# YuliangXiu/ICON

Measured on NVIDIA H100. Metric: M query-points/sec at 256^3 grid, higher is better.
Workload: dtype f32

## Files before the change

### icon_b200/_C.py

```python
import ctypes
import os

_HERE = os.path.dirname(os.path.abspath(__file__))
LIB_PATH = os.environ.get("ICON_B200_LIB") or os.path.join(_HERE, "libicon_b200.so")

if not os.path.exists(LIB_PATH):
    raise ImportError(
        f"{LIB_PATH} is missing: the CUDA extension must be built (python -m icon_b200.build); "
        "icon_b200 has no CPU or PyTorch fallback.")

lib = ctypes.CDLL(LIB_PATH)

_vp, _i, _i64, _f, _sz = ctypes.c_void_p, ctypes.c_int, ctypes.c_int64, ctypes.c_float, ctypes.c_size_t

_SIGS = {
    "icon_version": (_i, []),
    "icon_last_error": (ctypes.c_char_p, []),
    "icon_launch_count": (_i64, []),
    "icon_profile_enable": (_i, [_i]),
    "icon_profile_last_query": (_i, [_vp]),
    "icon_smpl_workspace_bytes": (_sz, [_i, _i]),
    "icon_smpl_prepare": (_i, [_vp, _vp, _vp, _vp, _i, _i, _vp, _sz, _vp]),
    "icon_query_workspace_bytes": (_sz, [_i64, _i, _i]),
    "icon_set_mlp_impl": (_i, [_i]),
    "icon_get_mlp_impl": (_i, []),
    "icon_query": (_i, [_i, _vp, _i64, _i64, _i64, _vp, _vp, _i, _i, _i, _vp, _i, _vp, _i, _i, _vp, _vp, _i, _f,
                        _vp, _vp, _sz, _vp]),
    "icon_query_feats": (_i, [_i, _vp, _i64, _i64, _i64, _vp, _vp, _i, _i, _i, _vp, _i, _vp, _i, _i, _vp, _vp, _i, _f,
                              _i, _vp, _vp, _sz, _vp]),
    "icon_set_sdf_policy": (_i, [_i, _i64, _i64]),
    "icon_set_sdf_bricks": (_i, [_i, _i64]),
    "icon_sdf_brick_info": (_i, [_vp, _i, _i, _vp]),
    "icon_sdf_brick_lists": (_i, [_vp, _i, _i, _vp, _vp, _vp, _vp, _vp, _vp, _vp]),
    "icon_sdf_only": (_i, [_vp, _i64, _i64, _i64, _vp, _vp, _i, _i, _vp, _vp, _vp, _sz, _vp]),
    "icon_sdf_bruteforce": (_i, [_vp, _i64, _i64, _i64, _vp, _vp, _i, _i, _vp, _vp, _vp]),
    "icon_mesh_workspace_bytes": (_sz, [_i, _i]),
    "icon_mesh_prepare": (_i, [_vp, _vp, _i, _i, _vp, _sz, _vp]),
    "icon_mesh_distance": (_i, [_vp, _i64, _vp, _i, _i, _vp, _vp, _vp]),
    "icon_mesh_sample_workspace_bytes": (_sz, [_i]),
    "icon_mesh_sample": (_i, [_vp, _vp, _i, _i, _vp, _i, ctypes.c_uint64, _vp, _vp, _vp, _vp, _sz, _vp]),
    "icon_prt_workspace_bytes": (_sz, [_i, _i, _i]),
    "icon_prt": (_i, [_vp, _i, _i, _vp, _vp, _i, ctypes.c_double, _vp, _vp, _i, _i, ctypes.c_double, _vp, _vp, _vp, _sz,
                      _vp]),
    "icon_mlp_only": (_i, [_vp, _i, _i64, _vp, _vp, _vp, _vp]),
# ... 135 lines not shown
```

### icon_b200/csrc/common.cu

```cuda
#include <stdarg.h>
#include <atomic>

#include <stdlib.h>

#include "common.cuh"

namespace icon {

static thread_local char g_err[512] = "";
static std::atomic<int64_t> g_launches{0};

void set_error(const char *fmt, ...) {
    va_list ap;
    va_start(ap, fmt);
    vsnprintf(g_err, sizeof(g_err), fmt, ap);
    va_end(ap);
}
void count_launch(int n) { g_launches += n; }

constexpr int SCAN_T = 1024, SCAN_I = 4, SCAN_B = SCAN_T * SCAN_I;

__global__ void __launch_bounds__(SCAN_T) k_scan_block(const int32_t *__restrict__ in,
                                                       int32_t *__restrict__ out, int64_t n,
                                                       int32_t *__restrict__ block_sums,
// ... 64 lines not shown
        return ICON_OK;
    }
    int64_t nb = (n + SCAN_B - 1) / SCAN_B;
    if (nb == 1) {
        k_scan_block<<<1, SCAN_T, 0, stream>>>(in, out, n, nullptr, d_total);
        ICON_LAUNCHED();
        return ICON_OK;
    }
    int32_t *sums = (int32_t *)ws;
    void *next_ws = (char *)ws + align_up((size_t)nb * sizeof(int32_t), 256);
    k_scan_block<<<(unsigned)nb, SCAN_T, 0, stream>>>(in, out, n, sums, nullptr);
    ICON_LAUNCHED();
    int rc = scan_exclusive_i32(sums, sums, nb, d_total, next_ws, stream);
    if (rc) return rc;
    k_scan_add<<<(unsigned)nb, SCAN_T, 0, stream>>>(out, n, sums);
    ICON_LAUNCHED();
    return ICON_OK;
}


__global__ void k_csr_count(const int32_t *__restrict__ own, int64_t n, int32_t *__restrict__ cnt) {
    const int64_t i = (int64_t)blockIdx.x * blockDim.x + threadIdx.x;
    if (i < n && own[i] >= 0) atomicAdd(&cnt[own[i]], 1);
}

__global__ void k_csr_fill(const int32_t *__restrict__ own, const int32_t *__restrict__ key, int64_t n,
                           const int32_t *__restrict__ off, int32_t *__restrict__ cursor, int32_t *__restrict__ list) {
    const int64_t i = (int64_t)blockIdx.x * blockDim.x + threadIdx.x;
    if (i < n && own[i] >= 0) list[off[own[i]] + atomicAdd(&cursor[own[i]], 1)] = key[i];
}
// ... 135 lines not shown
```

### icon_b200/csrc/common.cuh

```cuda
#pragma once
#include <cuda_runtime.h>
#include <stdint.h>
#include <stdio.h>

#include "../../include/icon_b200.h"

namespace icon {

void set_error(const char *fmt, ...);
void count_launch(int n = 1);

#define ICON_CHECK_ARG(cond, ...)                 \
    do {                                          \
        if (!(cond)) {                            \
            icon::set_error(__VA_ARGS__);         \
            return ICON_EINVAL;                   \
        }                                         \
    } while (0)

#define ICON_CUDA(expr)                                                              \
    do {                                                                             \
        cudaError_t _e = (expr);                                                     \
        if (_e != cudaSuccess) {                                                     \
            icon::set_error("%s:%d %s -> %s", __FILE__, __LINE__, #expr,             \
// ... 148 lines not shown
    unsigned short *flist;
    float *fkey;
    int64_t face_cap;
    int V;
};
size_t mesh_ws_bytes(int V, int F);
MeshView mesh_view(const void *ws, int V, int F);
void bricks_forget(const MeshView &m);

void profile_mark(int i, cudaStream_t stream);

size_t scan_ws_bytes(int64_t n);
int scan_exclusive_i32(const int32_t *in, int32_t *out, int64_t n, int64_t *d_total ,
                       void *ws, cudaStream_t stream);

struct CsrWs {
    int32_t *cnt, *cursor;
    void *scan_ws;
};
CsrWs csr_take(Carver &c, int64_t rows);
int csr_build(const int32_t *own, const int32_t *key, int64_t n, int R, int32_t *off, int32_t *list, int32_t *ucnt,
              const CsrWs &w, cudaStream_t stream);

size_t vertex_corners_ws_bytes(int V, int F);
int vertex_corners(const int64_t *faces, int F, int V, int32_t *off, int32_t *list, void *ws, cudaStream_t stream);

template <class Fn>
__device__ __forceinline__ void for_each_pass_corner(const int32_t *corners, int n, Fn &&fn) {
    for (int pass = 0; pass < 3; ++pass) {
        const int c = (pass + 1) % 3;
// ... 11 lines not shown
```

### icon_b200/csrc/mlp.cu

```cuda
#include "common.cuh"
#include "query_common.cuh"

namespace icon {

constexpr int MP = 64;
constexpr int MT = 256;
constexpr int KC = 16;

constexpr int OFF_W0 = 0;
constexpr int OFF_B0 = OFF_W0 + 16 * 512;
constexpr int OFF_W1 = OFF_B0 + 512;
constexpr int OFF_B1 = OFF_W1 + 512 * 256;
constexpr int OFF_W2 = OFF_B1 + 256;
constexpr int OFF_B2 = OFF_W2 + 272 * 128;
constexpr int OFF_W3 = OFF_B2 + 128;
constexpr int OFF_B3 = OFF_W3 + 144;
static_assert(OFF_B3 + 1 == ICON_MLP_PACKED_FLOATS, "packed layout");

template <int MODE>
__global__ void __launch_bounds__(MT, 2) k_query_mlp(QueryParams q) {
    extern __shared__ __align__(16) float sm[];
    float *x0s = sm;
    float *stage = sm + 16 * MP;
    float *h1s = stage + 10240;
// ... 213 lines not shown
    __syncthreads();
    if (tid < MP) {
        const int64_t pi = p0 + tid;
        if (pi < q.N) {
            float s = 0.f;
#pragma unroll
            for (int w = 0; w < 8; ++w) s += red[w * MP + tid];
            for (int j = 0; j < 16; ++j) s = fmaf(__ldg(W + OFF_W3 + 128 + j), x0s[j * MP + tid], s);
            s += __ldg(W + OFF_B3);
            float in_cube = (MODE == 3) ? 1.f : q.xyz4[pi].w;
            q.out[pi] = in_cube * s;
        }
    }
}

__global__ void k_outlier_flag(const float *__restrict__ rec, int64_t N, float clip, int32_t *__restrict__ flag) {
    int64_t i = (int64_t)blockIdx.x * blockDim.x + threadIdx.x;
    if (i < N) flag[i] = fabsf(rec[8 * i]) >= clip ? 1 : 0;
}
__global__ void k_outlier_signs(const float *__restrict__ rec, int64_t N, float clip,
                                const int32_t *__restrict__ krank, int8_t *__restrict__ signs) {
    int64_t i = (int64_t)blockIdx.x * blockDim.x + threadIdx.x;
    if (i < N) {
        float s = rec[8 * i];
        if (fabsf(s) >= clip) signs[krank[i]] = s > 0.f ? 1 : -1;
    }
}

constexpr size_t MLP_SMEM = (16 * MP + 10240 + 256 * MP) * sizeof(float);

template <int MODE>
static int launch_mlp(const QueryParams &q, cudaStream_t stream) {
    static bool attr_set[ICON_MAX_DEVICES] = {};
    if (device_needs_setup(attr_set))
        ICON_CUDA(cudaFuncSetAttribute(k_query_mlp<MODE>, cudaFuncAttributeMaxDynamicSharedMemorySize, (int)MLP_SMEM));
    unsigned nblk = (unsigned)((q.N + MP - 1) / MP);
    k_query_mlp<MODE><<<nblk, MT, MLP_SMEM, stream>>>(q);
    ICON_LAUNCHED();
    return ICON_OK;
}

int launch_mlp_tc(int mode, const QueryParams &q, const void *blob, cudaStream_t stream);
static int g_mlp_impl = 1;
// ... 5 lines not shown
            set_error("icon_query / icon_mlp_only: the tensor-core MLP needs the packed tensor-core weight blob (mlp_tc == NULL); "
                      "pass it or select the FP32 kernel with icon_set_mlp_impl(0)");
            return ICON_EINVAL;
        }
        if (q.c0 > 15) {
            set_error("icon_query / icon_mlp_only: the tensor-core MLP takes c0 <= 15 input channels (got %d)", q.c0);
            return ICON_EINVAL;
        }
        return launch_mlp_tc(MODE, q, tc, stream);
    }
    return launch_mlp<MODE>(q, stream);
}

size_t sdf_ws_bytes(int64_t N);
int run_sdf(const float *points, int64_t sc, int64_t sn, int64_t N, const float *h_calib, const MeshView &m,
            float *rec, int32_t *face, void *ws, float4 **xyz4_out, cudaStream_t stream);
int run_points_only(const float *points, int64_t sc, int64_t sn, int64_t N, const float *h_calib,
                    float4 *xyz4, cudaStream_t stream);

struct QueryWs {
    void *sdf_ws;
    float *rec;
    int32_t *krank;
    int8_t *signs;
    int64_t *d_K;
    void *scan_ws;
    float4 *xyz4;
};

static QueryWs carve_query(Carver &c, int64_t N, int prior) {
    QueryWs w{};
    if (prior == ICON_PRIOR_ICON) {
        w.sdf_ws = c.take<char>(sdf_ws_bytes(N));
        w.rec = c.take<float>((size_t)N * 8);
        w.krank = c.take<int32_t>((size_t)N);
        w.signs = c.take<int8_t>((size_t)N);
        w.d_K = c.take<int64_t>(1);
        w.scan_ws = c.take<char>(scan_ws_bytes(N));
    } else {
        w.xyz4 = c.take<float4>((size_t)N);
    }
    return w;
}

}

using namespace icon;

extern "C" size_t icon_query_workspace_bytes(int64_t N, int F, int prior) {
    (void)F;
    Carver c(nullptr);
    carve_query(c, N, prior);
    return c.total();
// ... 34 lines not shown
    q.feat = feat; q.C = C; q.H = H; q.W = W; q.vol = vol_feat; q.VD = VD;
    q.mlp = mlp_packed; q.c0 = c0; q.clip = sdf_clip; q.out = out; q.N = N;
    if (prior == ICON_PRIOR_ICON) {
        ICON_CHECK_ARG(mesh_ws && V > 0 && F > 0, "icon_query: icon prior needs a prepared body mesh");
        ICON_CHECK_ARG((smpl_feats & ~ICON_FEAT_ALL) == 0, "icon_query: smpl_feats mask %d has bits outside ICON_FEAT_ALL",
                       smpl_feats);
        const int cm = smpl_feats & ICON_FEAT_CMAP ? 1 : 0, nm = smpl_feats & ICON_FEAT_NORM ? 1 : 0;
        const bool vs = smpl_feats & ICON_FEAT_VIS;
        const int tail = 1 + 3 * cm + 3 * nm;
        ICON_CHECK_ARG((!vs || C % 2 == 0) && c0 == (vs ? C / 2 : C) + tail,
                       "icon_query: icon prior with smpl_feats mask %d expects c0 = %s + %d (C=%d c0=%d)", smpl_feats,
                       vs ? "C/2" : "C", tail, C, c0);
        q.feats = smpl_feats;
        MeshView m = mesh_view(mesh_ws, V, F);
        float4 *xyz4 = nullptr;
        int rc = run_sdf(points, stride_c, stride_n, N, h_calib, m, w.rec, nullptr, w.sdf_ws, &xyz4, stream);
        if (rc) return rc;
        if (cm) {
            unsigned nb = (unsigned)((N + 255) / 256);
            k_outlier_flag<<<nb, 256, 0, stream>>>(w.rec, N, sdf_clip, w.krank);
            ICON_LAUNCHED();
            rc = scan_exclusive_i32(w.krank, w.krank, N, w.d_K, w.scan_ws, stream);
            if (rc) return rc;
            k_outlier_signs<<<nb, 256, 0, stream>>>(w.rec, N, sdf_clip, w.krank, w.signs);
            ICON_LAUNCHED();
            q.krank = w.krank; q.signs = w.signs; q.d_K = w.d_K;
        }
        q.xyz4 = xyz4; q.rec = w.rec;
        profile_mark(3, stream);
        rc = launch_any<0>(q, mlp_tc, stream);
        profile_mark(4, stream);
        return rc;
    }
    profile_mark(0, stream);
    int rc = run_points_only(points, stride_c, stride_n, N, h_calib, w.xyz4, stream);
    if (rc) return rc;
    profile_mark(1, stream); profile_mark(2, stream); profile_mark(3, stream);
    q.xyz4 = w.xyz4;
    if (prior == ICON_PRIOR_PIFU) {
        ICON_CHECK_ARG(C + 1 == c0, "icon_query: pifu prior expects c0 = C + 1 (C=%d c0=%d)", C, c0);
        rc = launch_any<1>(q, mlp_tc, stream);
        profile_mark(4, stream);
        return rc;
    }
    if (prior == ICON_PRIOR_PAMIR) {
        ICON_CHECK_ARG(vol_feat && VD >= 2 && C + 7 == c0, "icon_query: pamir prior expects vol_feat and c0 = C + 7");
        rc = launch_any<2>(q, mlp_tc, stream);
        profile_mark(4, stream);
        return rc;
    }
    set_error("icon_query: unknown prior %d", prior);
    return ICON_EINVAL;
}

extern "C" int icon_set_mlp_impl(int impl) {
    ICON_CHECK_ARG(impl == 0 || impl == 1, "icon_set_mlp_impl: 0 (fp32) or 1 (tensor cores)");
    g_mlp_impl = impl;
    return ICON_OK;
}
extern "C" int icon_get_mlp_impl(void) { return g_mlp_impl; }

extern "C" int icon_mlp_only(const float *feature, int c0, int64_t N, const float *mlp_packed, const void *mlp_tc,
                             float *out, icon_stream_t stream_) {
    cudaStream_t stream = (cudaStream_t)stream_;
    if (N == 0) return ICON_OK;
    ICON_CHECK_ARG(feature && mlp_packed && out && c0 >= 1 && c0 <= 16, "icon_mlp_only: bad argument");
    QueryParams q{};
    q.raw = feature; q.mlp = mlp_packed; q.c0 = c0; q.out = out; q.N = N;
    return launch_any<3>(q, mlp_tc, stream);
// ... 2 lines not shown
```

### icon_b200/csrc/sdf.cu

```cuda
#include <float.h>

#include <algorithm>
#include <mutex>
#include <type_traits>
#include <unordered_set>
#include <vector>

#include "common.cuh"
#include "face_tree.cuh"
#include "geom.cuh"

namespace icon {

struct Calib {
    float r[9];
    float t[3];
};

__device__ __forceinline__ V3 load_point(const float *__restrict__ pts, int64_t sc, int64_t sn,
                                         int64_t i, const Calib &cb) {
    float px = pts[i * sn], py = pts[sc + i * sn], pz = pts[2 * sc + i * sn];
    V3 o;
    o.x = fmaf(cb.r[2], pz, fmaf(cb.r[1], py, cb.r[0] * px)) + cb.t[0];
    o.y = fmaf(cb.r[5], pz, fmaf(cb.r[4], py, cb.r[3] * px)) + cb.t[1];
    o.z = fmaf(cb.r[8], pz, fmaf(cb.r[7], py, cb.r[6] * px)) + cb.t[2];
    return o;
}

__device__ __forceinline__ void emit_record(V3 p, int bi, float best, int hits, const MeshView &m,
                                            float *__restrict__ rec, int32_t *__restrict__ face,
                                            int64_t idx) {
    Tri t = load_tri(m.tri + 3 * (size_t)bi);
    V3 n = cross3(t.ab, t.ac);
    float s = n.x * n.x + n.y * n.y + n.z * n.z;
    if (s == 0.f) s = 1e-6f;
    float inv = 1.0f / s;
    V3 w = sub3(p, t.a);
    V3 uw = cross3(t.ab, w), wv = cross3(w, t.ac);
    float b2 = (uw.x * n.x + uw.y * n.y + uw.z * n.z) * inv;
    float b1 = (wv.x * n.x + wv.y * n.y + wv.z * n.z) * inv;
    float b0 = 1.0f - b1 - b2;
    const float4 *at = m.attr + 6 * (size_t)bi;
    float4 a0 = __ldg(at), a1 = __ldg(at + 1), a2 = __ldg(at + 2), a3 = __ldg(at + 3),
           a4 = __ldg(at + 4), a5 = __ldg(at + 5);
    float nx = (a0.x * b0 + a0.w * b1 + a1.z * b2) * -1.f;
    float ny = (a0.y * b0 + a1.x * b1 + a1.w * b2) * 1.f;
    float nz = (a0.z * b0 + a1.y * b1 + a2.x * b2) * -1.f;
    float cx = a2.y * b0 + a3.x * b1 + a3.w * b2;
    float cy = a2.z * b0 + a3.y * b1 + a4.x * b2;
    float cz = a2.w * b0 + a3.z * b1 + a4.y * b2;
    float vv = a4.z * b0 + a4.w * b1 + a5.x * b2;
    float vis = vv >= 0.1f ? 1.f : 0.f;
    float dist = sqrtf(best) / sqrtf(3.0f);
    float sign = 2.0f * ((float)(hits & 1) - 0.5f);
    float sdf = dist * sign;
    float4 *r = (float4 *)(rec + 8 * idx);
    r[0] = make_float4(sdf, cx, cy, cz);
    r[1] = make_float4(nx, ny, nz, vis);
    if (face) face[idx] = bi;
}

constexpr int SW_T = 128;
constexpr int NBIN_AX = 128;
constexpr int NBIN = NBIN_AX * NBIN_AX * NBIN_AX;
__host__ __device__ constexpr int fr_cap(int ppw) { return ppw >= 16 ? 1024 : (ppw >= 4 ? 768 : 384); }

__device__ __forceinline__ unsigned spread7(unsigned v) {
    v = (v | (v << 16)) & 0x030000FFu;
    v = (v | (v << 8)) & 0x0300F00Fu;
    v = (v | (v << 4)) & 0x030C30C3u;
    v = (v | (v << 2)) & 0x09249249u;
    return v;
}

// ... 13 lines not shown
    int b = -1;
    if (live) {
        const V3 p = load_point(pts, sc, sn, i, cb);
        const float in_cube = (p.x > -1.f && p.x < 1.f && p.y > -1.f && p.y < 1.f && p.z > -1.f && p.z < 1.f) ? 1.f : 0.f;
        xyz4[i] = make_float4(p.x, p.y, p.z, in_cube);
        b = bin_of(p);
        bid[i] = b;
    }
    const unsigned act = __ballot_sync(0xffffffffu, live);
    if (live) {
        const unsigned peers = __match_any_sync(act, b);
        if ((int)(threadIdx.x & 31) == __ffs(peers) - 1) atomicAdd(&count[b], __popc(peers));
    }
}

__global__ void k_points_scatter(const int32_t *__restrict__ bid, int64_t N, const int32_t *__restrict__ offset,
                                 int32_t *__restrict__ cursor, int32_t *__restrict__ perm) {
    const int64_t i = (int64_t)blockIdx.x * blockDim.x + threadIdx.x;
    const bool live = i < N;
    const int b = live ? bid[i] : -1;
    const unsigned act = __ballot_sync(0xffffffffu, live);
    if (live) {
        const unsigned peers = __match_any_sync(act, b);
        const int lane = threadIdx.x & 31, leader = __ffs(peers) - 1;
        int base = 0;
        if (lane == leader) base = atomicAdd(&cursor[b], __popc(peers));
        base = __shfl_sync(peers, base, leader);
        perm[offset[b] + base + __popc(peers & ((1u << lane) - 1u))] = (int32_t)i;
    }
}

#ifdef ICON_SDF_STATS
__device__ unsigned long long g_stats[8];
__device__ unsigned *g_wstat;
enum { WS_DEFER, WS_ENTRIES, WS_STEPS, WS_STAGED, WS_SPH, WS_EXACT, WS_WIN, WS_RAY, WS_CYC_START, WS_CYC_C,
       WS_CYC_RAY, WS_CYC_EMIT, WS_UB0, WS_UBEND, WS_LIST, WS_IDEAL_ENTRIES, WS_IDEAL_FACES, WS_DEAD, WS_N = 20 };
#define STAT(i, v) do { if (lane == 0) atomicAdd(&g_stats[i], (unsigned long long)(v)); } while (0)
#define WSTAT(i, v) do { if (lane == 0 && g_wstat) g_wstat[(size_t)wid * WS_N + (i)] = (unsigned)(v); } while (0)
#define WCLK(t) __syncwarp(); const long long t = clock64()
#else
#define STAT(i, v) do { } while (0)
#define WSTAT(i, v) do { } while (0)
#endif
// ... 12 lines not shown
    hi = make_float4(-1.f + (bx + 1) * BRICK_W, -1.f + (by + 1) * BRICK_W, -1.f + (bz + 1) * BRICK_W, 0.f);
}

__device__ __forceinline__ float leaf_key(const MeshView &m, int l, float4 lo, float4 hi) {
    const float4 a = __ldg(m.nodes + 2 * (size_t)l), z = __ldg(m.nodes + 2 * (size_t)l + 1);
    const float gx = fmaxf(fmaxf(a.x - hi.x, lo.x - z.x), 0.f);
    const float gy = fmaxf(fmaxf(a.y - hi.y, lo.y - z.y), 0.f);
    const float gz = fmaxf(fmaxf(a.z - hi.z, lo.z - z.z), 0.f);
    return fmaf(gz, gz, fmaf(gy, gy, gx * gx));
}

template <int PPW, bool BRICK>
__device__ __forceinline__ void sdf_warp(int64_t wid, SdfSmem<PPW, BRICK> &S, const float4 *__restrict__ xyz4,
                                         const int32_t *__restrict__ perm, int64_t N, const MeshView &m,
                                         float *__restrict__ rec, int32_t *__restrict__ face,
                                         int32_t *__restrict__ defer, int32_t *__restrict__ ndefer) {
    constexpr int REP = 32 / PPW;
    const int lane = threadIdx.x & 31;
    const int sub = lane % PPW, rep_id = lane / PPW;
    const int64_t pos0 = wid * PPW;
    const int64_t pos = pos0 + sub;
    if (pos0 >= N) return;
    const bool live = pos < N;
    const int64_t idx = perm[live ? pos : pos0];
    const float4 q = xyz4[idx];
    const V3 p = mk3(q.x, q.y, q.z);
    const V3 c = mk3(0.5f * (warp_min(p.x) + warp_max(p.x)), 0.5f * (warp_min(p.y) + warp_max(p.y)),
                     0.5f * (warp_min(p.z) + warp_max(p.z)));
    const float rw = warp_max(sqrtf(dot3(sub3(p, c), sub3(p, c)))) * 1.00001f + 1e-6f;
    const float4 wlo = make_float4(warp_min(p.x) - 1e-6f, warp_min(p.y) - 1e-6f, warp_min(p.z) - 1e-6f, 0.f);
// ... 77 lines not shown
        }
    } else {
        for (int f = rep_id; f < m.F; f += REP) {
            const Tri tr = load_tri(m.tri + 3 * (size_t)f);
            hits += ray_hit_px(p, tr.a, tr.ab, tr.ac);
        }
    }
    if (REP > 1) {
#pragma unroll
        for (int o = PPW; o < 32; o <<= 1) hits += __shfl_xor_sync(0xffffffffu, hits, o);
    }
#ifdef ICON_SDF_STATS
    WCLK(t_ray0);
    t_ray = t_ray0;
#endif
    if (live && rep_id == 0) emit_record(p, nf.bi, nf.best, hits, m, rec, face, idx);
#ifdef ICON_SDF_STATS
    WCLK(t_end);
    if (BRICK && st_brick >= 0) {
        const float ube = nf.ub;
        int il = 0, ifc = 0;
        const int o0 = __ldg(m.foff + st_brick), o1 = __ldg(m.foff + st_brick + 1);
        for (int s = o0 + lane; s < o1; s += 32) {
            il += __ldg(m.fkey + s) <= ube * ube;
            const float4 s4 = __ldg(m.sph_s + __ldg(m.flist + s));
            const float l2 = ube + s4.w;
            ifc += box_dist2(mk3(s4.x, s4.y, s4.z), wlo, whi) <= l2 * l2;
        }
        const int s_sph = __reduce_add_sync(0xffffffffu, nf.n_sph), s_exact = __reduce_add_sync(0xffffffffu, nf.n_exact);
        const int s_win = __reduce_add_sync(0xffffffffu, nf.n_win), s_ray = __reduce_add_sync(0xffffffffu, st_ray);
        const int s_il = __reduce_add_sync(0xffffffffu, il), s_if = __reduce_add_sync(0xffffffffu, ifc);
// ... 10 lines not shown
        WSTAT(WS_CYC_EMIT, t_end - t_ray);
        WSTAT(WS_UB0, __float_as_uint(st_ub0));
        WSTAT(WS_UBEND, __float_as_uint(ube));
        WSTAT(WS_LIST, o1 - o0);
        WSTAT(WS_IDEAL_ENTRIES, s_il);
        WSTAT(WS_IDEAL_FACES, s_if);
        WSTAT(WS_DEAD, nf.n_dead);
    }
    if (!BRICK && defer != nullptr) { STAT(4, 1); STAT(5, t_end - t_start); }
#endif
}

template <int PPW, bool BRICK>
__global__ void __launch_bounds__(SW_T, PPW == 32 ? 8 : 0) k_sdf_warp(const float4 *__restrict__ xyz4, const int32_t *__restrict__ perm,
                                                   int64_t N, MeshView m, float *__restrict__ rec,
                                                   int32_t *__restrict__ face, int32_t *__restrict__ defer,
                                                   int32_t *__restrict__ ndefer) {
    static_assert(!BRICK || PPW == 32, "brick lists serve dense lattices: 32 points per warp");
    extern __shared__ __align__(16) unsigned char smem_raw[];
    SdfSmem<PPW, BRICK> &S = reinterpret_cast<SdfSmem<PPW, BRICK> *>(smem_raw)[threadIdx.x >> 5];
    const bool listed = !BRICK && defer != nullptr;
    const int64_t nw = listed ? (int64_t)*ndefer : (N + PPW - 1) / PPW;
    for (int64_t i = (int64_t)blockIdx.x * (SW_T / 32) + (threadIdx.x >> 5); i < nw; i += (int64_t)gridDim.x * (SW_T / 32))
        sdf_warp<PPW, BRICK>(listed ? (int64_t)defer[i] : i, S, xyz4, perm, N, m, rec, face, defer, ndefer);
}

__global__ void k_brick_centres(MeshView m) {
    const int b = blockIdx.x * blockDim.x + threadIdx.x;
    if (b >= NBRICK) return;
    float4 lo, hi;
    brick_box(b, lo, hi);
    m.bxyz[b] = make_float4(0.5f * (lo.x + hi.x), 0.5f * (lo.y + hi.y), 0.5f * (lo.z + hi.z), 0.f);
    m.bperm[b] = b;
}

template <class Take, class Put>
__device__ __forceinline__ int block_gather(int n, int *s_n, Take &&take, Put &&put) {
    __syncthreads();
    for (int i = threadIdx.x; i < n; i += blockDim.x) {
// ... 133 lines not shown
    for (int f0 = 0; f0 < m.F; f0 += 256) {
        int nf = min(256, m.F - f0);
        __syncthreads();
        for (int k = threadIdx.x; k < 3 * nf; k += 256) tile[k] = m.tri[3 * (size_t)f0 + k];
        __syncthreads();
        if (live) {
            for (int k = 0; k < nf; ++k) {
                float4 r0 = tile[3 * k], r1 = tile[3 * k + 1], r2 = tile[3 * k + 2];
                V3 a = mk3(r0.x, r0.y, r0.z), ab = mk3(r0.w, r1.x, r1.y), ac = mk3(r1.z, r1.w, r2.x);
                float d = tri_sqdist(p, a, ab, ac);
                if (d < best) { best = d; bi = f0 + k; }
                hits += ray_hit_px(p, a, ab, ac);
            }
        }
    }
    if (live) emit_record(p, bi, best, hits, m, rec, face, i);
}

static int64_t g_sdf_ppw32_from = 6000000, g_sdf_ppw8_from = 300000;
static int g_sdf_ppw_force = 0;
static int g_sdf_bricks = 1;
static int64_t g_brick_max_entries = 0;

static std::mutex g_brick_mu;
static std::unordered_set<const void *> g_brick_ready;
static int64_t g_brick_builds = 0;

void bricks_forget(const MeshView &m) {
    std::lock_guard<std::mutex> lk(g_brick_mu);
    g_brick_ready.erase(m.hdr);
}
// ... 10 lines not shown
    w.bid = c.take<int32_t>((size_t)N);
    w.perm = c.take<int32_t>((size_t)N);
    w.count = c.take<int32_t>(NBIN + 1);
    w.offset = c.take<int32_t>(NBIN + 1);
    w.defer = c.take<int32_t>((size_t)(N + 31) / 32);
    w.ndefer = c.take<int32_t>(1);
    w.scan_ws = c.take<char>(scan_ws_bytes(NBIN + 1));
    return w;
}

static int build_bricks(const MeshView &m, cudaStream_t stream) {
    const int64_t fcap = g_brick_max_entries > 0 ? std::min(g_brick_max_entries, m.face_cap) : m.face_cap;
    k_brick_centres<<<NBRICK / 256, 256, 0, stream>>>(m);
    ICON_LAUNCHED();
    k_sdf_warp<1, false><<<NBRICK / (SW_T / 32), SW_T, sdf_smem_bytes<1, false>(), stream>>>(
        m.bxyz, m.bperm, NBRICK, m, m.brec, m.bface, nullptr, nullptr);
    ICON_LAUNCHED();
    k_brick_faces<false><<<NBRICK, 128, 0, stream>>>(m, fcap);
    ICON_LAUNCHED();
    const int rc = scan_exclusive_i32(m.foff, m.foff, NBRICK + 1, nullptr, m.scan_ws, stream);
    if (rc) return rc;
    k_brick_faces<true><<<NBRICK, 128, 0, stream>>>(m, fcap);
    ICON_LAUNCHED();
    k_brick_done<<<1, 1, 0, stream>>>(m, fcap);
    ICON_LAUNCHED();
    return ICON_OK;
}
size_t sdf_ws_bytes(int64_t N) {
    Carver c(nullptr);
    carve_sdf(c, N);
    return c.total();
}

Calib make_calib(const float *h) {
    Calib cb;
    for (int r = 0; r < 3; ++r) {
        for (int k = 0; k < 3; ++k) cb.r[3 * r + k] = h[4 * r + k];
        cb.t[r] = h[4 * r + 3];
    }
    return cb;
}

int run_sdf(const float *points, int64_t sc, int64_t sn, int64_t N, const float *h_calib,
            const MeshView &m, float *rec, int32_t *face, void *ws, float4 **xyz4_out,
            cudaStream_t stream) {
    Carver c(ws);
    SdfWs w = carve_sdf(c, N);
    Calib cb = make_calib(h_calib);
    profile_mark(0, stream);
    ICON_CUDA(cudaMemsetAsync(w.count, 0, sizeof(int32_t) * (NBIN + 1), stream));
    const unsigned nblk = (unsigned)((N + 255) / 256);
    k_points_bin<<<nblk, 256, 0, stream>>>(points, sc, sn, N, cb, w.xyz4, w.bid, w.count);
    ICON_LAUNCHED();
    int rc = scan_exclusive_i32(w.count, w.offset, NBIN + 1, nullptr, w.scan_ws, stream);
    if (rc) return rc;
    ICON_CUDA(cudaMemsetAsync(w.count, 0, sizeof(int32_t) * (NBIN + 1), stream));
    k_points_scatter<<<nblk, 256, 0, stream>>>(w.bid, N, w.offset, w.count, w.perm);
    ICON_LAUNCHED();
    static bool attr_set[ICON_MAX_DEVICES] = {};
    if (device_needs_setup(attr_set)) {
#define ICON_SDF_ATTR(P, B) ICON_CUDA(cudaFuncSetAttribute(k_sdf_warp<P, B>, cudaFuncAttributeMaxDynamicSharedMemorySize, \
                                                           (int)sdf_smem_bytes<P, B>()))
        ICON_SDF_ATTR(32, true); ICON_SDF_ATTR(32, false); ICON_SDF_ATTR(16, false); ICON_SDF_ATTR(8, false);
        ICON_SDF_ATTR(4, false); ICON_SDF_ATTR(2, false); ICON_SDF_ATTR(1, false);
#undef ICON_SDF_ATTR
    }
    profile_mark(1, stream);
    int ppw = N >= g_sdf_ppw32_from ? 32 : (N >= g_sdf_ppw8_from ? 8 : 1);
    if (g_sdf_ppw_force) ppw = g_sdf_ppw_force;
    const int wpb = SW_T / 32;
    const int64_t nwarps = (N + ppw - 1) / ppw;
    const unsigned nblk_w = (unsigned)((nwarps + wpb - 1) / wpb);
#define ICON_SDF_LAUNCH(P) k_sdf_warp<P, false><<<nblk_w, SW_T, sdf_smem_bytes<P, false>(), stream>>>( \
        w.xyz4, w.perm, N, m, rec, face, nullptr, nullptr)
    if (ppw == 32 && g_sdf_bricks) {
        bool build;
        {
            std::lock_guard<std::mutex> lk(g_brick_mu);
            build = g_brick_ready.insert(m.hdr).second;
        }
        if (build) {
            rc = build_bricks(m, stream);
            std::lock_guard<std::mutex> lk(g_brick_mu);
            if (rc) { g_brick_ready.erase(m.hdr); return rc; }
            ++g_brick_builds;
        }
        ICON_CUDA(cudaMemsetAsync(w.ndefer, 0, sizeof(int32_t), stream));
        k_sdf_warp<32, true><<<nblk_w, SW_T, sdf_smem_bytes<32, true>(), stream>>>(
            w.xyz4, w.perm, N, m, rec, face, w.defer, w.ndefer);
        ICON_LAUNCHED();
        const unsigned nblk_d = (unsigned)std::min<int64_t>(nblk_w, (int64_t)device_sm_count() * 16);
        k_sdf_warp<32, false><<<nblk_d, SW_T, sdf_smem_bytes<32, false>(), stream>>>(
            w.xyz4, w.perm, N, m, rec, face, w.defer, w.ndefer);
    } else {
        switch (ppw) {
            case 32: ICON_SDF_LAUNCH(32); break;
            case 16: ICON_SDF_LAUNCH(16); break;
            case 8: ICON_SDF_LAUNCH(8); break;
            case 4: ICON_SDF_LAUNCH(4); break;
            case 2: ICON_SDF_LAUNCH(2); break;
            default: ICON_SDF_LAUNCH(1); break;
        }
    }
#undef ICON_SDF_LAUNCH
    ICON_LAUNCHED();
    profile_mark(2, stream);
    if (xyz4_out) *xyz4_out = w.xyz4;
    return ICON_OK;
// ... 100 lines not shown
    return ICON_OK;
}

extern "C" int icon_sdf_only(const float *points, int64_t stride_c, int64_t stride_n, int64_t N,
                             const float *h_calib, const void *mesh_ws, int V, int F, float *rec,
                             int32_t *face, void *ws, size_t ws_bytes, icon_stream_t stream_) {
    cudaStream_t stream = (cudaStream_t)stream_;
    ICON_CHECK_ARG(N >= 0 && N < (int64_t)INT32_MAX, "icon_sdf_only: N=%lld out of range", (long long)N);
    if (N == 0) return ICON_OK;
    ICON_CHECK_ARG(points && h_calib && mesh_ws && rec && ws, "icon_sdf_only: null pointer");
    if (ws_bytes < sdf_ws_bytes(N)) {
        set_error("icon_sdf_only: workspace %zu < %zu", ws_bytes, sdf_ws_bytes(N));
        return ICON_ENOSPC;
    }
    MeshView m = mesh_view(mesh_ws, V, F);
    return run_sdf(points, stride_c, stride_n, N, h_calib, m, rec, face, ws, nullptr, stream);
}

extern "C" int icon_sdf_bruteforce(const float *points, int64_t stride_c, int64_t stride_n, int64_t N,
                                   const float *h_calib, const void *mesh_ws, int V, int F, float *rec,
                                   int32_t *face, icon_stream_t stream_) {
    cudaStream_t stream = (cudaStream_t)stream_;
    if (N == 0) return ICON_OK;
    ICON_CHECK_ARG(points && h_calib && mesh_ws && rec, "icon_sdf_bruteforce: null pointer");
    MeshView m = mesh_view(mesh_ws, V, F);
    Calib cb = make_calib(h_calib);
    k_sdf_brute<<<(unsigned)((N + 255) / 256), 256, 0, stream>>>(points, stride_c, stride_n, N, cb, m, rec, face);
    ICON_LAUNCHED();
    return ICON_OK;
}
```

### icon_b200/ops.py

```python
import ctypes

import torch

from . import _C
from ._C import check, lib

PRIOR_ID = {"icon": 0, "pifu": 1, "pamir": 2}
MLP_PACKED_FLOATS = 16 * 512 + 512 + 512 * 256 + 256 + 272 * 128 + 128 + 144 + 1


def _stream():
    return ctypes.c_void_p(torch.cuda.current_stream().cuda_stream)


def _p(t):
    return ctypes.c_void_p(t.data_ptr()) if t is not None else ctypes.c_void_p(0)


def _need_cuda(*ts):
    for t in ts:
        if t is not None and not t.is_cuda:
            raise _C.IconError("icon_b200 ops need CUDA tensors: there is no CPU path")


# ... 182 lines not shown
    unknown = set(smpl_feats) - set(_FEAT_BIT)
    if unknown:
        raise _C.IconError(f"smpl_feats: unknown feature(s) {sorted(unknown)}; the icon prior knows {list(SMPL_FEATS_ALL)}")
    mask = 0
    for name in set(smpl_feats):
        mask |= _FEAT_BIT[name]
    return mask


def icon_c0(smpl_feats, C):
    mask = smpl_feats_mask(smpl_feats)
    return (C // 2 if mask & FEAT_VIS else C) + 1 + 3 * bool(mask & FEAT_CMAP) + 3 * bool(mask & FEAT_NORM)


def query(prior, points, calib, feat, mlp, c0=None, body=None, vol_feat=None, sdf_clip=0.05, out=None,
          smpl_feats=SMPL_FEATS_ALL):
    _need_cuda(points, feat, mlp.f32, mlp.tc, vol_feat)
    c0 = mlp.c0
    pts, sc, sn, N = _point_strides(points)
    feat = feat.detach()
    if feat.dim() != 4 or feat.shape[0] != 1:
        raise _C.IconError(f"feature map must be [1,C,H,W], got {tuple(feat.shape)}")
    feat = feat.float().contiguous()
    C, H, W = feat.shape[1:]
    mask = smpl_feats_mask(smpl_feats) if prior == "icon" else 0
    pid = PRIOR_ID[prior]
    if out is None:
        out = torch.empty(1, 1, N, dtype=torch.float32, device=pts.device)
    V = F = 0
    mesh = None
    if prior == "icon":
        if body is None:
            raise _C.IconError("icon prior needs a prepared SmplBody")
        V, F, mesh = body.V, body.F, body.ws
    VD = 0
    if prior == "pamir":
        vol_feat = vol_feat.detach().float().contiguous()
        if vol_feat.dim() != 5 or vol_feat.shape[0] != 1 or vol_feat.shape[1] != 7 or \
                not (vol_feat.shape[2] == vol_feat.shape[3] == vol_feat.shape[4]):
            raise _C.IconError(f"vol_feat must be [1,7,D,D,D], got {tuple(vol_feat.shape)}")
        VD = vol_feat.shape[2]
    nbytes = lib.icon_query_workspace_bytes(N, F, pid)
    ws = torch.empty(max(nbytes, 256), dtype=torch.uint8, device=pts.device)
    check(lib.icon_query_feats(pid, _p(pts), sc, sn, N, _calib_rows(calib), _p(feat), C, H, W, _p(vol_feat), VD,
                               _p(mesh), V, F, _p(mlp.f32), _p(mlp.tc), c0, float(sdf_clip), mask, _p(out), _p(ws),
                               nbytes, _stream()),
          "icon_query")
    return out


def sdf_only(points, calib, body, brute=False):
    _need_cuda(points)
    pts, sc, sn, N = _point_strides(points)
    rec = torch.empty(N, 8, dtype=torch.float32, device=pts.device)
    face = torch.empty(N, dtype=torch.int32, device=pts.device)
    if brute:
        check(lib.icon_sdf_bruteforce(_p(pts), sc, sn, N, _calib_rows(calib), _p(body.ws), body.V, body.F, _p(rec),
                                      _p(face), _stream()), "icon_sdf_bruteforce")
    else:
        nbytes = lib.icon_query_workspace_bytes(N, body.F, 0)
        ws = torch.empty(max(nbytes, 256), dtype=torch.uint8, device=pts.device)
        check(lib.icon_sdf_only(_p(pts), sc, sn, N, _calib_rows(calib), _p(body.ws), body.V, body.F, _p(rec),
# ... 139 lines not shown
```

### include/icon_b200.h

```cpp
#ifndef ICON_B200_H
#define ICON_B200_H

#include <stddef.h>
#include <stdint.h>

#ifdef __cplusplus
extern "C" {
#endif

#define ICON_OK 0
#define ICON_EINVAL (-1)
#define ICON_ECUDA (-2)
#define ICON_ENOSPC (-3)

#define ICON_PRIOR_ICON 0
#define ICON_PRIOR_PIFU 1
#define ICON_PRIOR_PAMIR 2

typedef void *icon_stream_t;

int icon_version(void);
const char *icon_last_error(void);
int64_t icon_launch_count(void);

// ... 14 lines not shown
int icon_query(int prior, const float *points, int64_t stride_c, int64_t stride_n, int64_t N,
               const float *h_calib, const float *feat, int C, int H, int W,
               const float *vol_feat, int VD, const void *mesh_ws, int V, int F,
               const float *mlp_packed, const void *mlp_tc, int c0, float sdf_clip, float *out,
               void *ws, size_t ws_bytes, icon_stream_t stream);

#define ICON_FEAT_CMAP 1
#define ICON_FEAT_NORM 2
#define ICON_FEAT_VIS 4
#define ICON_FEAT_ALL (ICON_FEAT_CMAP | ICON_FEAT_NORM | ICON_FEAT_VIS)
int icon_query_feats(int prior, const float *points, int64_t stride_c, int64_t stride_n, int64_t N,
                     const float *h_calib, const float *feat, int C, int H, int W,
                     const float *vol_feat, int VD, const void *mesh_ws, int V, int F,
                     const float *mlp_packed, const void *mlp_tc, int c0, float sdf_clip, int smpl_feats,
                     float *out, void *ws, size_t ws_bytes, icon_stream_t stream);

int icon_set_sdf_policy(int force_ppw, int64_t ppw8_from, int64_t ppw32_from);
int icon_set_sdf_bricks(int enable, int64_t max_entries);
int icon_sdf_brick_info(const void *mesh_ws, int V, int F, int64_t *out);
int icon_sdf_brick_lists(const void *mesh_ws, int V, int F, int64_t *dims, int32_t *foff, int32_t *flist,
                         float *fkey, float *bub, int32_t *bface, float *sph);

int icon_sdf_only(const float *points, int64_t stride_c, int64_t stride_n, int64_t N,
                  const float *h_calib, const void *mesh_ws, int V, int F, float *rec,
                  int32_t *face, void *ws, size_t ws_bytes, icon_stream_t stream);
int icon_sdf_bruteforce(const float *points, int64_t stride_c, int64_t stride_n, int64_t N,
                        const float *h_calib, const void *mesh_ws, int V, int F, float *rec,
                        int32_t *face, icon_stream_t stream);
size_t icon_mesh_workspace_bytes(int V, int F);
int icon_mesh_prepare(const float *verts, const int64_t *faces, int V, int F, void *mesh_ws, size_t mesh_ws_bytes,
// ... 250 lines not shown
```

Measured before the change: 629.9.

## Fuse outlier classification into SDF emit and replace per-point scan with block rank

The SDF kernel now writes a one-byte outlier class per point (inside, outside, or neither) when it emits each record. A new two-pass block count, scan and rank computes the compacted outlier ranks and signs from these bytes. This replaces the separate flag kernel, the full-length int32 scan and the sign kernel, which each re-read the 32-byte rec rows. Point scattering also reuses the offset array as its atomic cursor, which drops a memset. A debug export API and a caller-supplied workspace option are added as well.

```diff
diff --git a/icon_b200/_C.py b/icon_b200/_C.py
--- a/icon_b200/_C.py
+++ b/icon_b200/_C.py
@@ -28,6 +28,7 @@
                         _vp, _vp, _sz, _vp]),
     "icon_query_feats": (_i, [_i, _vp, _i64, _i64, _i64, _vp, _vp, _i, _i, _i, _vp, _i, _vp, _i, _i, _vp, _vp, _i, _f,
                               _i, _vp, _vp, _sz, _vp]),
+    "icon_query_outlier_rank": (_i, [_vp, _i64, _vp, _vp, _vp, _vp, _vp]),
     "icon_set_sdf_policy": (_i, [_i, _i64, _i64]),
     "icon_set_sdf_bricks": (_i, [_i, _i64]),
     "icon_sdf_brick_info": (_i, [_vp, _i, _i, _vp]),
diff --git a/icon_b200/csrc/common.cu b/icon_b200/csrc/common.cu
--- a/icon_b200/csrc/common.cu
+++ b/icon_b200/csrc/common.cu
@@ -102,6 +102,117 @@
     int rc = scan_exclusive_i32(sums, sums, nb, d_total, next_ws, stream);
     if (rc) return rc;
     k_scan_add<<<(unsigned)nb, SCAN_T, 0, stream>>>(out, n, sums);
+    ICON_LAUNCHED();
+    return ICON_OK;
+}
+
+constexpr int FR_T = 256, FR_I = 16, FR_B = FR_T * FR_I;
+
+__device__ __forceinline__ void load_classes(const uint8_t *__restrict__ cls, int64_t base, int64_t n,
+                                             uint8_t (&c)[FR_I]) {
+    if (base + FR_I <= n) {
+        const uint4 v = *(const uint4 *)(cls + base);
+        const unsigned w[4] = {v.x, v.y, v.z, v.w};
+#pragma unroll
+        for (int i = 0; i < FR_I; ++i) c[i] = (uint8_t)(w[i / 4] >> (8 * (i % 4)));
+    } else {
+#pragma unroll
+        for (int i = 0; i < FR_I; ++i) c[i] = base + i < n ? cls[base + i] : 0;
+    }
+}
+
+__device__ __forceinline__ int count_nonzero(const uint8_t (&c)[FR_I]) {
+    int s = 0;
+#pragma unroll
+    for (int i = 0; i < FR_I; ++i) s += c[i] != 0;
+    return s;
+}
+
+__global__ void __launch_bounds__(FR_T) k_class_count(const uint8_t *__restrict__ cls, int64_t n,
+                                                      int32_t *__restrict__ bcnt) {
+    __shared__ int32_t warp_tot[FR_T / 32];
+    uint8_t c[FR_I];
+    load_classes(cls, (int64_t)blockIdx.x * FR_B + (int64_t)threadIdx.x * FR_I, n, c);
+    const int s = __reduce_add_sync(0xffffffffu, (unsigned)count_nonzero(c));
+    if ((threadIdx.x & 31) == 0) warp_tot[threadIdx.x >> 5] = s;
+    __syncthreads();
+    if (threadIdx.x == 0) {
+        int t = 0;
+#pragma unroll
+        for (int w = 0; w < FR_T / 32; ++w) t += warp_tot[w];
+        bcnt[blockIdx.x] = t;
+    }
+}
+
+__global__ void __launch_bounds__(FR_T) k_class_rank(const uint8_t *__restrict__ cls, int64_t n,
+                                                     const int32_t *__restrict__ boff, int32_t *__restrict__ rank,
+                                                     int8_t *__restrict__ sign) {
+    __shared__ int32_t warp_off[FR_T / 32];
+    const int lane = threadIdx.x & 31, wid = threadIdx.x >> 5;
+    const int64_t base = (int64_t)blockIdx.x * FR_B + (int64_t)threadIdx.x * FR_I;
+    uint8_t c[FR_I];
+    load_classes(cls, base, n, c);
+    const int s = count_nonzero(c);
+    int incl = s;
+#pragma unroll
+    for (int o = 1; o < 32; o <<= 1) {
+        const int t = __shfl_up_sync(0xffffffffu, incl, o);
+        if (lane >= o) incl += t;
+    }
+    if (lane == 31) warp_off[wid] = incl;
+    __syncthreads();
+    if (wid == 0) {
+        const int w = lane < FR_T / 32 ? warp_off[lane] : 0;
+        int wi = w;
+#pragma unroll
+        for (int o = 1; o < FR_T / 32; o <<= 1) {
+            const int t = __shfl_up_sync(0xffffffffu, wi, o);
+            if (lane >= o) wi += t;
+        }
+        if (lane < FR_T / 32) warp_off[lane] = boff[blockIdx.x] + wi - w;
+    }
+    __syncthreads();
+    int r = warp_off[wid] + incl - s;
+    int32_t out[FR_I];
+#pragma unroll
+    for (int i = 0; i < FR_I; ++i) {
+        out[i] = r;
+        if (c[i]) {
+            if (sign) sign[r] = c[i] == 1 ? 1 : -1;
+            ++r;
+        }
+    }
+    if (base + FR_I <= n) {
+#pragma unroll
+        for (int i = 0; i < FR_I; i += 4) *(int4 *)(rank + base + i) = make_int4(out[i], out[i + 1], out[i + 2], out[i + 3]);
+    } else {
+#pragma unroll
+        for (int i = 0; i < FR_I; ++i)
+            if (base + i < n) rank[base + i] = out[i];
+    }
+}
+
+static int64_t class_rank_blocks(int64_t n) { return (n + FR_B - 1) / FR_B; }
+
+size_t class_rank_ws_bytes(int64_t n) {
+    const int64_t nb = class_rank_blocks(n);
+    return align_up((size_t)nb * sizeof(int32_t), 256) + scan_ws_bytes(nb);
+}
+
+int class_rank(const uint8_t *cls, int64_t n, int32_t *rank, int8_t *sign, int64_t *d_total, void *ws,
+               cudaStream_t stream) {
+    if (n <= 0) {
+        ICON_CUDA(cudaMemsetAsync(d_total, 0, sizeof(int64_t), stream));
+        return ICON_OK;
+    }
+    const int64_t nb = class_rank_blocks(n);
+    int32_t *boff = (int32_t *)ws;
+    void *scan_ws = (char *)ws + align_up((size_t)nb * sizeof(int32_t), 256);
+    k_class_count<<<(unsigned)nb, FR_T, 0, stream>>>(cls, n, boff);
+    ICON_LAUNCHED();
+    const int rc = scan_exclusive_i32(boff, boff, nb, d_total, scan_ws, stream);
+    if (rc) return rc;
+    k_class_rank<<<(unsigned)nb, FR_T, 0, stream>>>(cls, n, boff, rank, sign);
     ICON_LAUNCHED();
     return ICON_OK;
 }
diff --git a/icon_b200/csrc/common.cuh b/icon_b200/csrc/common.cuh
--- a/icon_b200/csrc/common.cuh
+++ b/icon_b200/csrc/common.cuh
@@ -186,6 +186,10 @@
 int scan_exclusive_i32(const int32_t *in, int32_t *out, int64_t n, int64_t *d_total ,
                        void *ws, cudaStream_t stream);
 
+size_t class_rank_ws_bytes(int64_t n);
+int class_rank(const uint8_t *cls, int64_t n, int32_t *rank, int8_t *sign, int64_t *d_total, void *ws,
+               cudaStream_t stream);
+
 struct CsrWs {
     int32_t *cnt, *cursor;
     void *scan_ws;
diff --git a/icon_b200/csrc/mlp.cu b/icon_b200/csrc/mlp.cu
--- a/icon_b200/csrc/mlp.cu
+++ b/icon_b200/csrc/mlp.cu
@@ -251,19 +251,6 @@
     }
 }
 
-__global__ void k_outlier_flag(const float *__restrict__ rec, int64_t N, float clip, int32_t *__restrict__ flag) {
-    int64_t i = (int64_t)blockIdx.x * blockDim.x + threadIdx.x;
-    if (i < N) flag[i] = fabsf(rec[8 * i]) >= clip ? 1 : 0;
-}
-__global__ void k_outlier_signs(const float *__restrict__ rec, int64_t N, float clip,
-                                const int32_t *__restrict__ krank, int8_t *__restrict__ signs) {
-    int64_t i = (int64_t)blockIdx.x * blockDim.x + threadIdx.x;
-    if (i < N) {
-        float s = rec[8 * i];
-        if (fabsf(s) >= clip) signs[krank[i]] = s > 0.f ? 1 : -1;
-    }
-}
-
 constexpr size_t MLP_SMEM = (16 * MP + 10240 + 256 * MP) * sizeof(float);
 
 template <int MODE>
@@ -299,7 +286,7 @@
 
 size_t sdf_ws_bytes(int64_t N);
 int run_sdf(const float *points, int64_t sc, int64_t sn, int64_t N, const float *h_calib, const MeshView &m,
-            float *rec, int32_t *face, void *ws, float4 **xyz4_out, cudaStream_t stream);
+            float *rec, int32_t *face, float clip, uint8_t *cls, void *ws, float4 **xyz4_out, cudaStream_t stream);
 int run_points_only(const float *points, int64_t sc, int64_t sn, int64_t N, const float *h_calib,
                     float4 *xyz4, cudaStream_t stream);
 
@@ -309,7 +296,8 @@
     int32_t *krank;
     int8_t *signs;
     int64_t *d_K;
-    void *scan_ws;
+    uint8_t *cls;
+    void *rank_ws;
     float4 *xyz4;
 };
 
@@ -321,7 +309,8 @@
         w.krank = c.take<int32_t>((size_t)N);
         w.signs = c.take<int8_t>((size_t)N);
         w.d_K = c.take<int64_t>(1);
-        w.scan_ws = c.take<char>(scan_ws_bytes(N));
+        w.cls = c.take<uint8_t>((size_t)N);
+        w.rank_ws = c.take<char>(class_rank_ws_bytes(N));
     } else {
         w.xyz4 = c.take<float4>((size_t)N);
     }
@@ -386,16 +375,12 @@
         q.feats = smpl_feats;
         MeshView m = mesh_view(mesh_ws, V, F);
         float4 *xyz4 = nullptr;
-        int rc = run_sdf(points, stride_c, stride_n, N, h_calib, m, w.rec, nullptr, w.sdf_ws, &xyz4, stream);
+        int rc = run_sdf(points, stride_c, stride_n, N, h_calib, m, w.rec, nullptr, sdf_clip, cm ? w.cls : nullptr,
+                         w.sdf_ws, &xyz4, stream);
         if (rc) return rc;
         if (cm) {
-            unsigned nb = (unsigned)((N + 255) / 256);
-            k_outlier_flag<<<nb, 256, 0, stream>>>(w.rec, N, sdf_clip, w.krank);
-            ICON_LAUNCHED();
-            rc = scan_exclusive_i32(w.krank, w.krank, N, w.d_K, w.scan_ws, stream);
+            rc = class_rank(w.cls, N, w.krank, w.signs, w.d_K, w.rank_ws, stream);
             if (rc) return rc;
-            k_outlier_signs<<<nb, 256, 0, stream>>>(w.rec, N, sdf_clip, w.krank, w.signs);
-            ICON_LAUNCHED();
             q.krank = w.krank; q.signs = w.signs; q.d_K = w.d_K;
         }
         q.xyz4 = xyz4; q.rec = w.rec;
@@ -425,6 +410,24 @@
     return ICON_EINVAL;
 }
 
+extern "C" int icon_query_outlier_rank(const void *ws, int64_t N, int64_t *K, int32_t *krank, int8_t *signs,
+                                       uint8_t *cls, float *rec) {
+    ICON_CHECK_ARG(ws && K && N > 0 && N < (int64_t)INT32_MAX, "icon_query_outlier_rank: bad argument");
+    Carver c((void *)ws);
+    const QueryWs w = carve_query(c, N, ICON_PRIOR_ICON);
+    ICON_CUDA(cudaDeviceSynchronize());
+    ICON_CUDA(cudaMemcpy(K, w.d_K, sizeof(int64_t), cudaMemcpyDeviceToHost));
+    if (krank) ICON_CUDA(cudaMemcpy(krank, w.krank, sizeof(int32_t) * N, cudaMemcpyDeviceToHost));
+    if (signs) {
+        ICON_CHECK_ARG(*K >= 0 && *K <= N, "icon_query_outlier_rank: K=%lld outside [0, N]: no rank in this workspace",
+                       (long long)*K);
+        ICON_CUDA(cudaMemcpy(signs, w.signs, (size_t)*K, cudaMemcpyDeviceToHost));
+    }
+    if (cls) ICON_CUDA(cudaMemcpy(cls, w.cls, N, cudaMemcpyDeviceToHost));
+    if (rec) ICON_CUDA(cudaMemcpy(rec, w.rec, sizeof(float) * 8 * N, cudaMemcpyDeviceToHost));
+    return ICON_OK;
+}
+
 extern "C" int icon_set_mlp_impl(int impl) {
     ICON_CHECK_ARG(impl == 0 || impl == 1, "icon_set_mlp_impl: 0 (fp32) or 1 (tensor cores)");
     g_mlp_impl = impl;
diff --git a/icon_b200/csrc/sdf.cu b/icon_b200/csrc/sdf.cu
--- a/icon_b200/csrc/sdf.cu
+++ b/icon_b200/csrc/sdf.cu
@@ -29,7 +29,7 @@
 
 __device__ __forceinline__ void emit_record(V3 p, int bi, float best, int hits, const MeshView &m,
                                             float *__restrict__ rec, int32_t *__restrict__ face,
-                                            int64_t idx) {
+                                            uint8_t *__restrict__ cls, float clip, int64_t idx) {
     Tri t = load_tri(m.tri + 3 * (size_t)bi);
     V3 n = cross3(t.ab, t.ac);
     float s = n.x * n.x + n.y * n.y + n.z * n.z;
@@ -58,6 +58,7 @@
     r[0] = make_float4(sdf, cx, cy, cz);
     r[1] = make_float4(nx, ny, nz, vis);
     if (face) face[idx] = bi;
+    if (cls) cls[idx] = fabsf(sdf) >= clip ? (sdf > 0.f ? 1 : 2) : 0;
 }
 
 constexpr int SW_T = 128;
@@ -101,8 +102,8 @@
     }
 }
 
-__global__ void k_points_scatter(const int32_t *__restrict__ bid, int64_t N, const int32_t *__restrict__ offset,
-                                 int32_t *__restrict__ cursor, int32_t *__restrict__ perm) {
+__global__ void k_points_scatter(const int32_t *__restrict__ bid, int64_t N, int32_t *__restrict__ offset,
+                                 int32_t *__restrict__ perm) {
     const int64_t i = (int64_t)blockIdx.x * blockDim.x + threadIdx.x;
     const bool live = i < N;
     const int b = live ? bid[i] : -1;
@@ -111,9 +112,9 @@
         const unsigned peers = __match_any_sync(act, b);
         const int lane = threadIdx.x & 31, leader = __ffs(peers) - 1;
         int base = 0;
-        if (lane == leader) base = atomicAdd(&cursor[b], __popc(peers));
+        if (lane == leader) base = atomicAdd(&offset[b], __popc(peers));
         base = __shfl_sync(peers, base, leader);
-        perm[offset[b] + base + __popc(peers & ((1u << lane) - 1u))] = (int32_t)i;
+        perm[base + __popc(peers & ((1u << lane) - 1u))] = (int32_t)i;
     }
 }
 
@@ -156,6 +157,7 @@
 __device__ __forceinline__ void sdf_warp(int64_t wid, SdfSmem<PPW, BRICK> &S, const float4 *__restrict__ xyz4,
                                          const int32_t *__restrict__ perm, int64_t N, const MeshView &m,
                                          float *__restrict__ rec, int32_t *__restrict__ face,
+                                         uint8_t *__restrict__ cls, float clip,
                                          int32_t *__restrict__ defer, int32_t *__restrict__ ndefer) {
     constexpr int REP = 32 / PPW;
     const int lane = threadIdx.x & 31;
@@ -263,7 +265,7 @@
     WCLK(t_ray0);
     t_ray = t_ray0;
 #endif
-    if (live && rep_id == 0) emit_record(p, nf.bi, nf.best, hits, m, rec, face, idx);
+    if (live && rep_id == 0) emit_record(p, nf.bi, nf.best, hits, m, rec, face, cls, clip, idx);
 #ifdef ICON_SDF_STATS
     WCLK(t_end);
     if (BRICK && st_brick >= 0) {
@@ -304,15 +306,15 @@
 template <int PPW, bool BRICK>
 __global__ void __launch_bounds__(SW_T, PPW == 32 ? 8 : 0) k_sdf_warp(const float4 *__restrict__ xyz4, const int32_t *__restrict__ perm,
                                                    int64_t N, MeshView m, float *__restrict__ rec,
-                                                   int32_t *__restrict__ face, int32_t *__restrict__ defer,
-                                                   int32_t *__restrict__ ndefer) {
+                                                   int32_t *__restrict__ face, uint8_t *__restrict__ cls, float clip,
+                                                   int32_t *__restrict__ defer, int32_t *__restrict__ ndefer) {
     static_assert(!BRICK || PPW == 32, "brick lists serve dense lattices: 32 points per warp");
     extern __shared__ __align__(16) unsigned char smem_raw[];
     SdfSmem<PPW, BRICK> &S = reinterpret_cast<SdfSmem<PPW, BRICK> *>(smem_raw)[threadIdx.x >> 5];
     const bool listed = !BRICK && defer != nullptr;
     const int64_t nw = listed ? (int64_t)*ndefer : (N + PPW - 1) / PPW;
     for (int64_t i = (int64_t)blockIdx.x * (SW_T / 32) + (threadIdx.x >> 5); i < nw; i += (int64_t)gridDim.x * (SW_T / 32))
-        sdf_warp<PPW, BRICK>(listed ? (int64_t)defer[i] : i, S, xyz4, perm, N, m, rec, face, defer, ndefer);
+        sdf_warp<PPW, BRICK>(listed ? (int64_t)defer[i] : i, S, xyz4, perm, N, m, rec, face, cls, clip, defer, ndefer);
 }
 
 __global__ void k_brick_centres(MeshView m) {
@@ -476,7 +478,7 @@
             }
         }
     }
-    if (live) emit_record(p, bi, best, hits, m, rec, face, i);
+    if (live) emit_record(p, bi, best, hits, m, rec, face, nullptr, 0.f, i);
 }
 
 static int64_t g_sdf_ppw32_from = 6000000, g_sdf_ppw8_from = 300000;
@@ -517,7 +519,7 @@
     k_brick_centres<<<NBRICK / 256, 256, 0, stream>>>(m);
     ICON_LAUNCHED();
     k_sdf_warp<1, false><<<NBRICK / (SW_T / 32), SW_T, sdf_smem_bytes<1, false>(), stream>>>(
-        m.bxyz, m.bperm, NBRICK, m, m.brec, m.bface, nullptr, nullptr);
+        m.bxyz, m.bperm, NBRICK, m, m.brec, m.bface, nullptr, 0.f, nullptr, nullptr);
     ICON_LAUNCHED();
     k_brick_faces<false><<<NBRICK, 128, 0, stream>>>(m, fcap);
     ICON_LAUNCHED();
@@ -545,7 +547,7 @@
 }
 
 int run_sdf(const float *points, int64_t sc, int64_t sn, int64_t N, const float *h_calib,
-            const MeshView &m, float *rec, int32_t *face, void *ws, float4 **xyz4_out,
+            const MeshView &m, float *rec, int32_t *face, float clip, uint8_t *cls, void *ws, float4 **xyz4_out,
             cudaStream_t stream) {
     Carver c(ws);
     SdfWs w = carve_sdf(c, N);
@@ -557,8 +559,7 @@
     ICON_LAUNCHED();
     int rc = scan_exclusive_i32(w.count, w.offset, NBIN + 1, nullptr, w.scan_ws, stream);
     if (rc) return rc;
-    ICON_CUDA(cudaMemsetAsync(w.count, 0, sizeof(int32_t) * (NBIN + 1), stream));
-    k_points_scatter<<<nblk, 256, 0, stream>>>(w.bid, N, w.offset, w.count, w.perm);
+    k_points_scatter<<<nblk, 256, 0, stream>>>(w.bid, N, w.offset, w.perm);
     ICON_LAUNCHED();
     static bool attr_set[ICON_MAX_DEVICES] = {};
     if (device_needs_setup(attr_set)) {
@@ -575,7 +576,7 @@
     const int64_t nwarps = (N + ppw - 1) / ppw;
     const unsigned nblk_w = (unsigned)((nwarps + wpb - 1) / wpb);
 #define ICON_SDF_LAUNCH(P) k_sdf_warp<P, false><<<nblk_w, SW_T, sdf_smem_bytes<P, false>(), stream>>>( \
-        w.xyz4, w.perm, N, m, rec, face, nullptr, nullptr)
+        w.xyz4, w.perm, N, m, rec, face, cls, clip, nullptr, nullptr)
     if (ppw == 32 && g_sdf_bricks) {
         bool build;
         {
@@ -590,11 +591,11 @@
         }
         ICON_CUDA(cudaMemsetAsync(w.ndefer, 0, sizeof(int32_t), stream));
         k_sdf_warp<32, true><<<nblk_w, SW_T, sdf_smem_bytes<32, true>(), stream>>>(
-            w.xyz4, w.perm, N, m, rec, face, w.defer, w.ndefer);
+            w.xyz4, w.perm, N, m, rec, face, cls, clip, w.defer, w.ndefer);
         ICON_LAUNCHED();
         const unsigned nblk_d = (unsigned)std::min<int64_t>(nblk_w, (int64_t)device_sm_count() * 16);
         k_sdf_warp<32, false><<<nblk_d, SW_T, sdf_smem_bytes<32, false>(), stream>>>(
-            w.xyz4, w.perm, N, m, rec, face, w.defer, w.ndefer);
+            w.xyz4, w.perm, N, m, rec, face, cls, clip, w.defer, w.ndefer);
     } else {
         switch (ppw) {
             case 32: ICON_SDF_LAUNCH(32); break;
@@ -725,7 +726,7 @@
         return ICON_ENOSPC;
     }
     MeshView m = mesh_view(mesh_ws, V, F);
-    return run_sdf(points, stride_c, stride_n, N, h_calib, m, rec, face, ws, nullptr, stream);
+    return run_sdf(points, stride_c, stride_n, N, h_calib, m, rec, face, 0.f, nullptr, ws, nullptr, stream);
 }
 
 extern "C" int icon_sdf_bruteforce(const float *points, int64_t stride_c, int64_t stride_n, int64_t N,
diff --git a/icon_b200/ops.py b/icon_b200/ops.py
--- a/icon_b200/ops.py
+++ b/icon_b200/ops.py
@@ -220,7 +220,7 @@
 
 
 def query(prior, points, calib, feat, mlp, c0=None, body=None, vol_feat=None, sdf_clip=0.05, out=None,
-          smpl_feats=SMPL_FEATS_ALL):
+          smpl_feats=SMPL_FEATS_ALL, ws=None):
     _need_cuda(points, feat, mlp.f32, mlp.tc, vol_feat)
     c0 = mlp.c0
     pts, sc, sn, N = _point_strides(points)
@@ -247,11 +247,34 @@
             raise _C.IconError(f"vol_feat must be [1,7,D,D,D], got {tuple(vol_feat.shape)}")
         VD = vol_feat.shape[2]
     nbytes = lib.icon_query_workspace_bytes(N, F, pid)
-    ws = torch.empty(max(nbytes, 256), dtype=torch.uint8, device=pts.device)
+    if ws is None:
+        ws = torch.empty(max(nbytes, 256), dtype=torch.uint8, device=pts.device)
+    else:
+        _need_cuda(ws)
+        if ws.dtype != torch.uint8 or not ws.is_contiguous() or ws.numel() < nbytes:
+            raise _C.IconError(f"ws must be a contiguous uint8 tensor of at least {nbytes} bytes")
+        nbytes = ws.numel()
     check(lib.icon_query_feats(pid, _p(pts), sc, sn, N, _calib_rows(calib), _p(feat), C, H, W, _p(vol_feat), VD,
                                _p(mesh), V, F, _p(mlp.f32), _p(mlp.tc), c0, float(sdf_clip), mask, _p(out), _p(ws),
                                nbytes, _stream()),
           "icon_query")
+    return out
+
+
+def query_workspace_bytes(N, prior="icon"):
+    return int(lib.icon_query_workspace_bytes(int(N), 0, PRIOR_ID[prior]))
+
+
+def query_outlier_rank(ws, N):
+    K = ctypes.c_int64()
+    check(lib.icon_query_outlier_rank(_p(ws), int(N), ctypes.byref(K), None, None, None, None), "icon_query_outlier_rank")
+    out = {"krank": torch.empty(N, dtype=torch.int32), "cls": torch.empty(N, dtype=torch.uint8),
+           "rec": torch.empty(N, 8, dtype=torch.float32)}
+    out["signs"] = torch.empty(K.value if 0 <= K.value <= N else 0, dtype=torch.int8)
+    check(lib.icon_query_outlier_rank(_p(ws), int(N), ctypes.byref(K), _p(out["krank"]),
+                                      _p(out["signs"]) if 0 <= K.value <= N else None, _p(out["cls"]), _p(out["rec"])),
+          "icon_query_outlier_rank")
+    out["K"] = int(K.value)
     return out
 
 
diff --git a/include/icon_b200.h b/include/icon_b200.h
--- a/include/icon_b200.h
+++ b/include/icon_b200.h
@@ -52,6 +52,9 @@
                      const float *vol_feat, int VD, const void *mesh_ws, int V, int F,
                      const float *mlp_packed, const void *mlp_tc, int c0, float sdf_clip, int smpl_feats,
                      float *out, void *ws, size_t ws_bytes, icon_stream_t stream);
+
+int icon_query_outlier_rank(const void *ws, int64_t N, int64_t *K, int32_t *krank, int8_t *signs, uint8_t *cls,
+                            float *rec);
 
 int icon_set_sdf_policy(int force_ppw, int64_t ppw8_from, int64_t ppw32_from);
 int icon_set_sdf_bricks(int enable, int64_t max_entries);
```

Measured after the change: 637.5 (median of 6 runs). +1.2%, better.
